# mryndzionek/composable-sdr

Measured on AMD Instinct MI355X. Metric: MS/s CF32 throughput, 256-ch PFB+FM pipeline, higher is better.
Workload: dtype f32; 1 GPU; cfg3: 256-ch firpfbch(m=7,As=80)+dcBlocker+freqdem(kf=0.3) on synthetic CF32, AGC off (-a 0), 262144 frames/step (512 MiB in, 256 MiB out), HBM-resident; channels=256, demod=fm, mix=False, route=fused-256|k_tile256<FM>, preheat_steps=12094, collective=none, rccl_ranks=1

## Files before the change

composable_sdr_amd/csrc/fused_common.h:

```cpp
#pragma once
#include "fused.h"
#include "run_split.h"

#include <cmath>
#include <cstdlib>
#include <vector>

namespace csdr {
namespace {

constexpr int M256 = 256;
constexpr int P = 14;
constexpr int NB = 16;
constexpr int FS_X = 272;
constexpr int FS_Z = 289;
constexpr int RS_Z = 18;
constexpr int RS_Y = 17;
constexpr int LDS_F2 = 16 * FS_Z;
constexpr int E_OFF = 4096;
constexpr int LOOKBACK = 10;
constexpr unsigned SPIN_LIMIT = 1u << 24;

typedef unsigned long long u64;
typedef float v2f __attribute__((ext_vector_type(2)));
// ... 327 lines not shown
    return f ? r : make_float2(0.f, 0.f);
}


constexpr int WU = 6;


struct RunArgs {
    TileArgs t;
    RunSplit split;
    PhaseK pk;
    uint32_t nruns;
    float l2beta;
    uint32_t prio_div;
    uint32_t trace_light;
    const float4 *prev_tail;
    uint32_t indep;
    uint32_t pair_align;
    uint32_t wu_batch6;
    uint32_t wu, wu_rot;
    uint32_t tile_step;
    uint32_t nowu;
    float2 *cpre, *side;
};
constexpr int DCFIX_F = 113;

__device__ __forceinline__ float2 wg_sum(float2 v, float2 *red, int tid)
{
#pragma unroll
    for (int d = 32; d >= 1; d >>= 1) { v.x += __shfl_xor(v.x, d); v.y += __shfl_xor(v.y, d); }
    if ((tid & 63) == 0) red[tid >> 6] = v;
    __syncthreads();
    const float2 r = cadd(cadd(red[0], red[1]), cadd(red[2], red[3]));
    __syncthreads();
    return r;
}

__device__ __forceinline__ void row_scan4(float &x0, float &x1, float &x2, float &x3, float &s0, float &s1, float &s2, float &s3,
                                          float b1, float b2, float b4, float b8, float na)
{
    asm volatile(
        "v_mov_b32_e32 %4, %0\n\t"
        "v_mov_b32_e32 %5, %1\n\t"
        "v_mov_b32_e32 %6, %2\n\t"
        "v_mov_b32_e32 %7, %3\n\t"
        "v_fmac_f32_dpp %4, %4, %8 row_shr:1 row_mask:0xf bank_mask:0xf\n\t"
        "v_fmac_f32_dpp %5, %5, %8 row_shr:1 row_mask:0xf bank_mask:0xf\n\t"
        "v_fmac_f32_dpp %6, %6, %8 row_shr:1 row_mask:0xf bank_mask:0xf\n\t"
// ... 72 lines not shown
```

composable_sdr_amd/csrc/fused_v2_common.h:

```cpp
#pragma once
#include "fused_common.h"

namespace csdr {
namespace {

typedef float v4f __attribute__((ext_vector_type(4)));
#ifndef V2_DMA_AUX
#define V2_DMA_AUX ""
#endif
#ifndef V2_DMA_AUX_STREAM
#define V2_DMA_AUX_STREAM V2_DMA_AUX
#endif

__device__ __forceinline__ void bar()
{
    asm volatile("s_waitcnt lgkmcnt(0)\n\ts_barrier" ::: "memory");
}
__device__ __forceinline__ float opaque_v(float x) { asm volatile("" : "+v"(x)); return x; }

__device__ __forceinline__ unsigned dma_offset(int tid)
{
    const int wave = tid >> 6, lane = tid & 63;
    const int slot = 64 * wave + lane, q = slot >> 3, i = (slot & 7) ^ ((q >> 1) & 7);
    return (unsigned)(8 * q + i) * 16u;
// ... 107 lines not shown
    const v2f wA = piv - uA, wB = piv - uB;
    m[0] = copysignf(sel_neg(q[0].x, wA.x, uA.x), q[0].y);
    m[1] = copysignf(sel_neg(q[1].x, wA.y, uA.y), q[1].y);
    m[2] = copysignf(sel_neg(q[2].x, wB.x, uB.x), q[2].y);
    m[3] = copysignf(sel_neg(q[3].x, wB.y, uB.y), q[3].y);
}

template <int CTRL> __device__ __forceinline__ float dpp_keep(float old, float v)
{
    return __int_as_float(__builtin_amdgcn_update_dpp(__float_as_int(old), __float_as_int(v), CTRL, 0xf, 0xf, false));
}

}
template <size_t OFF> __device__ __forceinline__ unsigned kernarg_u32_s()
{
    unsigned v = 0;
#if defined(__HIP_DEVICE_COMPILE__)
    typedef __attribute__((address_space(4))) const char *kptr;
    kptr ka = (kptr)__builtin_amdgcn_kernarg_segment_ptr();
    asm volatile("s_load_dword %0, %1, %2\n\ts_waitcnt lgkmcnt(0)" : "=s"(v) : "s"(ka), "n"(OFF) : "memory");
#endif
    return v;
}
template <size_t OFF> __device__ __forceinline__ float2 *kernarg_ptr_s()
{
    float2 *p = nullptr;
#if defined(__HIP_DEVICE_COMPILE__)
    typedef __attribute__((address_space(4))) const char *kptr;
    kptr ka = (kptr)__builtin_amdgcn_kernarg_segment_ptr();
    unsigned long long v;
    asm volatile("s_load_dwordx2 %0, %1, %2\n\ts_waitcnt lgkmcnt(0)" : "=s"(v) : "s"(ka), "n"(OFF) : "memory");
    p = reinterpret_cast<float2 *>(v);
#endif
    return p;
}

}
```

composable_sdr_amd/csrc/kernels_fused.hip:

```cpp
#include "fused_common.h"
#include <cstring>

namespace csdr {

namespace {

#define STAMP(i) do { if (A.trace && tid == 0) A.trace[(size_t)b * 16 + (i)] = __builtin_amdgcn_s_memtime(); } while (0)

template <bool FM>
__global__ __launch_bounds__(256) void k_tile256(TileArgs A)
{
    __shared__ __attribute__((aligned(16))) float2 R[LDS_F2];
    __shared__ float2 tw_s[M256];
    __shared__ float2 Tt[2][16];
    __shared__ float2 carry_s[2];
    __shared__ unsigned tile_s;

    const int tid = threadIdx.x;
    if (tid == 0) tile_s = atomicAdd(A.ticket, 1u);
    tw_s[tid] = A.tw[tid];
    __syncthreads();
    const unsigned b = tile_s;
    if (b >= A.nb) return;
    STAMP(0);
// ... 247 lines not shown

__global__ __launch_bounds__(64) void k_shard_gather(const float *__restrict__ src, float *__restrict__ dst, uint32_t c0, uint32_t G, uint32_t rem,
                                                     uint32_t nf, uint32_t t0, uint32_t w)
{
    const uint32_t m = blockIdx.x;
    for (uint32_t i = threadIdx.x; i < rem * w; i += 64) dst[((size_t)m * nf + t0) * w + i] = src[(size_t)(c0 + G * m) * rem * w + i];
}

constexpr float V2_WEIGHT_CF[8] = {1.2f, 0.8f, 1.f, 1.f, 1.f, 1.f, 1.f, 1.f};
constexpr float V2_WEIGHT_FM[8] = {1.24f, 0.76f, 1.f, 1.f, 1.f, 1.f, 1.f, 1.f};
constexpr float V2_WEIGHT_FM3[8] = {1.6f, 1.f, 0.6f, 1.f, 1.f, 1.f, 1.f, 1.f};
constexpr float EQUAL_WEIGHT[8] = {1.f, 1.f, 1.f, 1.f, 1.f, 1.f, 1.f, 1.f};

struct FusedPlan : ChainPlan {
    using ChainPlan::ChainPlan;
    std::string kernel;
    uint32_t max_nb = 0, epoch = 0;
    float *d_taps = nullptr;
    float2 *d_tw = nullptr, *d_wpre = nullptr;
    StreamState st;
    unsigned *d_ticket = nullptr, *d_yflag = nullptr, *d_status = nullptr;
    u64 *d_agg = nullptr, *d_ylast = nullptr;
    ColdStart cold;
    u64 *d_trace = nullptr;
    uint32_t run_min_tiles = 1024;
    float slot_weight[8] = {1.f, 1.f, 1.f, 1.f, 1.f, 1.f, 1.f, 1.f};
    uint32_t slot_pairs[8] = {0, 0, 0, 0, 0, 0, 0, 0};
    bool have_weights = false, have_pairs = false;
    bool pd_equal = false, pd_nocopy = false;
    uint32_t resident_wgs_v2 = 512;
    float *d_shard_tail = nullptr;
    float4 *d_tail[3] = {nullptr, nullptr, nullptr};
    int tail_w = 0;
    bool tail_valid = false, save_tails = false;
    TileArgs proto;
    RunArgs run_proto;

    int init();
    const char *name() const override { return kernel.c_str(); }
    bool tile_major_ok(uint32_t nf) const override;
    void keep_tail() override { save_tails = cfg.G == 1; }
    bool can_overlap(uint32_t nf) const override;
    bool tail_recorded() const override { return save_tails && tail_valid; }
    int status(unsigned *st) override;
    int trace(unsigned long long *out, uint32_t ntiles) override;
    int reset_state(hipStream_t s) override;
// ... 32 lines not shown
    if ((r = mem.alloc(&d_ticket, sizeof(unsigned)))) return r;
    if ((r = mem.alloc(&d_status, sizeof(unsigned)))) return r;
    if ((r = mem.alloc(&d_yflag, sizeof(unsigned) * max_nb))) return r;
    if ((r = mem.alloc(&d_agg, sizeof(u64) * 2 * max_nb))) return r;
    if ((r = mem.alloc(&d_ylast, sizeof(u64) * (size_t)cfg.M * max_nb))) return r;
    if (const char *e = diag_env("CSDR_RUN_MIN_TILES")) run_min_tiles = (uint32_t)atol(e);
    if (cfg.mix && (r = mem.alloc(&d_premix, (size_t)cfg.C * cfg.max_nf * (cfg.fm ? 4 : 8)))) return r;
    const char *trace_knob = diag_env("CSDR_TRACE");
    if (trace_knob) {
        if ((r = mem.alloc(&d_trace, sizeof(u64) * 16 * max_nb))) return r;
        CSDR_HIP(hipMemset(d_trace, 0, sizeof(u64) * 16 * max_nb));
    }
    CSDR_HIP(hipMemcpy(d_taps, cfg.taps, sizeof(float) * cfg.M * cfg.p, hipMemcpyHostToDevice));
    std::vector<float2> tw(cfg.M);
    for (uint32_t k1 = 0; k1 < 16; k1++)
        for (uint32_t b1 = 0; b1 < 16; b1++) {
            const double a = -2.0 * 3.14159265358979323846 * (double)(b1 * k1) / (double)cfg.M;
            tw[16 * k1 + b1] = make_float2((float)std::cos(a), (float)std::sin(a));
        }
    const std::vector<float2> wpre = premix_table();
    CSDR_HIP(hipMemcpy(d_tw, tw.data(), sizeof(float2) * cfg.M, hipMemcpyHostToDevice));
    CSDR_HIP(hipMemcpy(d_wpre, wpre.data(), sizeof(float2) * 2 * cfg.M, hipMemcpyHostToDevice));
    if (cfg.G == 1 && cfg.c0 == 0 && cfg.C == cfg.M &&
        (r = cold.init(mem, cfg, (DCFIX_F - 1) * 256.0, 2050, (size_t)2048 * 4 * DCFIX_F, false, 15u, (uint32_t)DCFIX_F, 126, wpre.data()))) return r;
    CSDR_HIP(hipMemset(d_status, 0, sizeof(unsigned)));
    CSDR_HIP(hipMemset(d_yflag, 0, sizeof(unsigned) * max_nb));
    CSDR_HIP(hipMemset(d_agg, 0, sizeof(u64) * 2 * max_nb));

    TileArgs &A = proto;
    A = TileArgs{};
    A.taps = d_taps; A.tw = d_tw; A.wpre = d_wpre;
    A.ticket = d_ticket; A.agg = d_agg; A.ylast = d_ylast; A.yflag = d_yflag; A.status = d_status;
    A.c0 = cfg.c0; A.C = cfg.C; A.fm_ref = cfg.fm_ref; A.trace = d_trace;
    dcc.put(A);
    if (const char *e = diag_env("CSDR_CUS")) { if (atoi(e) > 0 && (uint32_t)atoi(e) < cus) cus = (uint32_t)atoi(e); }
    resident_wgs_v2 = (uint32_t)(cus * run256_v2_blocks_per_cu(cfg.fm, cfg.G));
    if (const char *e = diag_env("CSDR_RESIDENT_WGS")) resident_wgs_v2 = (uint32_t)atol(e);
    if (const char *e = diag_env("CSDR_RUN_WEIGHTS")) { parse_list(e, slot_weight, atof); have_weights = true; }
    if (const char *e = diag_env("CSDR_RUN_PAIRS")) { parse_list(e, slot_pairs, atol); have_pairs = true; }
    pd_equal = diag_env("CSDR_PD_EQUAL") != nullptr;
    pd_nocopy = diag_env("CSDR_PD_NOCOPY") != nullptr;

    RunArgs &RA = run_proto;
    RA = RunArgs{};
    RA.pk = phase_consts(cfg.fm_ref);
    RA.l2beta = dcc.l2beta;
    RA.cpre = cold.cpre; RA.side = cold.side;
    { const char *e = diag_env("CSDR_PRIO_ROT"); RA.prio_div = (e && atoi(e)) ? cus : 0u; }
    RA.trace_light = (trace_knob && atoi(trace_knob) == 2) ? 1u : 0u;
    { const char *e = diag_env("CSDR_WU"); RA.wu = e ? (uint32_t)atoi(e) : (uint32_t)WU; }
    { const char *e = diag_env("CSDR_WU_ROT"); RA.wu_rot = e ? (uint32_t)atoi(e) : 0u; }
    RA.pair_align = (cfg.fm || diag_env("CSDR_PAIR_ALIGN_CF")) ? 1u : 0u;
    { const char *e = diag_env("CSDR_WU_BATCH6"); RA.wu_batch6 = e ? (uint32_t)atoi(e) : 1u; }
    return 0;
}

int FusedPlan::reset_state(hipStream_t s)
{
    if (int r = st.reset(s)) return r;
    CSDR_HIP(hipMemsetAsync(d_tail[0], 0, sizeof(float4) * 2048 * (WU + 1), s));
    tail_w = 0; tail_valid = true;
    return 0;
}

bool FusedPlan::tile_major_ok(uint32_t nf) const
{
    if (cfg.fm || cfg.mix || nf % NB || !nf) return false;
    if (cfg.G > 1) return (uint64_t)cfg.C * nf * 8u < (1ull << 32);
    return cfg.c0 == 0 && cfg.C == cfg.M && nf / NB >= run_min_tiles;
}

bool FusedPlan::can_overlap(uint32_t nf) const
{
    return save_tails && tail_valid && v2_call(nf) && nf % NB == 0 && !cfg.mix;
}

void FusedPlan::wire_state(TileArgs &A) const
{
    A.yhist_in = st.hist_in(cur); A.yhist_out = st.hist_out(cur);
    A.vend_in = st.vend_in(cur);  A.vend_out = st.vend_out(cur);
    A.rp_in = st.rp_in(cur);      A.rp_out = st.rp_out(cur);
}
// ... 25 lines not shown
    CSDR_HIP(hipGetLastError());
    return 0;
}

int FusedPlan::run_kernel(const FusedCall &call, const TileArgs &A, hipStream_t s, KernelTimer *timer)
{
    const FusedConfig &c = cfg;
    const bool shard = c.G > 1;
    int r;
    kernel = c.fm ? "k_run256v2<FM>" : "k_run256v2<CF32>";
    if (shard) kernel += "/G" + std::to_string(c.G);
    RunArgs RA = run_proto;
    RA.t = A;
    uint32_t nruns = resident_wgs_v2;
    if (nruns > A.nb / 8) nruns = A.nb / 8;
    if (nruns < 1) nruns = 1;
    RA.nruns = nruns;
    const float *v2_weight = c.fm ? ((cus && nruns == 3 * cus) ? V2_WEIGHT_FM3 : V2_WEIGHT_FM) : V2_WEIGHT_CF;
    RA.split = make_split(A.nb, nruns, cus, (call.indep && pd_equal) ? EQUAL_WEIGHT : (have_weights ? slot_weight : v2_weight),
                          have_pairs ? slot_pairs : nullptr);
    RA.tile_step = call.tile_major ? c.C * 128u : (uint32_t)NB * (c.fm ? 4u : 8u);
    RA.indep = call.indep ? 1u : 0u;
    RA.nowu = (cold.rt && !shard && !RA.indep && nruns >= 2 && nruns <= 2048) ? 1u : 0u;
    RA.prev_tail = d_tail[tail_w];
    if (save_tails && !shard && call.nf == A.nb * NB && A.nb >= WU + 1) {
        const int nxt = (tail_w + 1) % 3;
        if (!pd_nocopy) hipLaunchKernelGGL(k_save_tail, dim3(2048 * (WU + 1) / 256), dim3(256), 0, s,
                                           reinterpret_cast<const float4 *>(call.d_in + (size_t)(A.nb - (WU + 1)) * 4096), d_tail[nxt]);
        if (call.ev_tail) CSDR_HIP(hipEventRecord(call.ev_tail, s));
        tail_w = nxt; tail_valid = true;
    } else tail_valid = false;
    if (timer && (r = timer->begin(s))) return r;
    if (A.nb && (r = run256_v2_launch(&RA, c.fm, c.G, nruns, s))) return r;
    if (RA.nowu && A.nb && (r = run256_dcfix_launch(&RA, c.fm, nruns, cold.rt, s))) return r;
    if (timer && (r = timer->end(s))) return r;
    return 0;
}

int FusedPlan::tile_kernel(TileArgs &T, hipStream_t s, KernelTimer *timer)
{
    int r;
    if (++epoch == 0) epoch = 1;
    T.epoch = epoch;
    CSDR_HIP(hipMemsetAsync(d_ticket, 0, sizeof(unsigned), s));
    if (timer && (r = timer->begin(s))) return r;
    if (cfg.fm) hipLaunchKernelGGL(k_tile256<true>, dim3(T.nb), dim3(256), 0, s, T);
    else hipLaunchKernelGGL(k_tile256<false>, dim3(T.nb), dim3(256), 0, s, T);
    if (timer && (r = timer->end(s))) return r;
    return 0;
}

int FusedPlan::ragged_end(const FusedCall &call, void *out, uint32_t nb_full, uint32_t rem, hipStream_t s)
{
    const FusedConfig &c = cfg;
    const bool shard = c.G > 1;
    int r;
    if (nb_full) cur ^= 1;
    TileArgs T = proto;
// ... 30 lines not shown
```

composable_sdr_amd/csrc/kernels_fused_v2.hip:

```cpp
#ifndef V2_FM_PACKED
#define V2_FM_PACKED 1
#endif
#ifndef V2_ABLATE
#define V2_ABLATE 0
#endif

#ifndef V2_COLSCAN
#define V2_COLSCAN 0
#endif
#ifndef V2_PAIR
#define V2_PAIR 1
#endif
#ifndef V2_STORE_AUX
#define V2_STORE_AUX ""
#endif
#ifndef V2_PAIR_CF
#define V2_PAIR_CF 0
#endif
#ifndef V2_BAR_E
#define V2_BAR_E 0
#endif
#ifndef V2_PAD
#define V2_PAD 1
#endif
// ... 10 lines not shown
#include "fused_v2_common.h"
#include <cstddef>
#include <type_traits>

namespace csdr {
namespace {

constexpr unsigned V2_FSB = 2048u + (V2_PAD ? 128u : 0u);
constexpr int V2_FS2 = (int)V2_FSB / 8;
constexpr int V2_BUF = 16 * V2_FS2;
constexpr int V2_STASH = 2 * V2_BUF;
constexpr int V2_AUX2 = 256 + 32 + 256 + (V2_COLSCAN ? 512 : 0);
constexpr int V2_F2 = V2_STASH + V2_AUX2;
constexpr int V2_F2_ONE = V2_BUF + V2_AUX2 + P * M256 / 2;
#define V2_ZSW(f) (V2_PAD ? (((f) >> 1) & 7) : ((f) & 7))
#ifndef V2_RSWN
#define V2_RSWN V2_PAD
#endif
#define V2_RSW(a) (V2_RSWN ? ((a) & 7) : (((a) >> 1) & 7))

struct V2Args {
    RunArgs r;
};

template <bool FM, int G>
__global__ __launch_bounds__(256, (FM && G == 1) ? V2_ONE_WGS : 2) void k_run256v2(V2Args VA)
{
    static_assert(G == 1 || G == 2 || G == 4 || G == 8, "interleaved shards: G = 2, 4, 8");
    constexpr int NK1 = 16 / G;
    constexpr bool ONE = FM && G == 1;
    const RunArgs &RA = VA.r;
    const TileArgs &A = RA.t;
    __shared__ __attribute__((aligned(16))) float2 L[(ONE && V2_ONE_WGS >= 3) ? V2_F2_ONE : V2_F2];
    float2 *R = L, *ST = L + (ONE ? V2_BUF : V2_STASH), *Tt = ST + 256, *red = Tt + 16;
    float2 *tw_s = red + 16;
    float2 *TRc = tw_s + 256, *Ec = TRc + 256;
    (void)TRc; (void)Ec;
    float *TP = reinterpret_cast<float *>(L + (ONE ? V2_BUF : V2_STASH) + V2_AUX2);
    float2 *H = ONE ? L : L + V2_BUF;
    float2 *HS = ONE ? reinterpret_cast<float2 *>(TP) : H;
    float2 *E = ST;
    const int tid = threadIdx.x, j = tid;
    const unsigned w = blockIdx.x;
    unsigned first, last;
    run_range(RA.split, w, first, last);
    if (RA.pair_align) {
// ... 22 lines not shown
    const bool cold = w > 0 || RA.indep;
    const int halo = (int)first - 1;
    auto tile_ptr = [&](int t) -> const float4 * { return t >= 0 ? x4 + (size_t)t * 2048 : RA.prev_tail + (size_t)(WU + 1 + t) * 2048; };
    if (ONE) {
        if (cold) dma_tile<false, 2 * V2_FSB>(tile_ptr(halo), goff, lds_wave);
        else if (first < last) dma_tile<false, 2 * V2_FSB>(x4 + (size_t)first * 2048, goff, lds_wave);
    } else {
        if (first < last) dma_tile<false, 2 * V2_FSB>(x4 + (size_t)first * 2048, goff, lds_wave);
        if (cold) dma_tile<false, 2 * V2_FSB>(tile_ptr(halo), goff, lds_wave + (unsigned)(V2_BUF * 8));
    }
    float h[P];
#pragma unroll
    for (int n = 0; n < P; n++) h[n] = A.taps[(M256 - 1 - j) + n * M256];
    float2 Wa = A.wpre[(A.parity0 & 1) * M256 + j], Wb = A.wpre[((A.parity0 & 1) ^ 1) * M256 + j];
    if (G > 1) {
        const int n = ((j >> 4) * (int)A.c0) & 15;
        const float C1 = 0.92387953251128674f, S1 = 0.38268343236508977f, R2 = 0.70710678118654752f;
        const int m4 = n & 3, qd = n >> 2;
        const float2 e = m4 == 0 ? make_float2(1.f, 0.f) : (m4 == 1 ? make_float2(C1, -S1) : (m4 == 2 ? make_float2(R2, -R2) : make_float2(S1, -C1)));
        const float2 rot = qd == 0 ? e : (qd == 1 ? make_float2(e.y, -e.x) : (qd == 2 ? make_float2(-e.x, -e.y) : make_float2(-e.y, e.x)));
        Wa = cmul(Wa, rot); Wb = cmul(Wb, rot);
    }
    tw_s[tid] = A.tw[tid];
    float2 wa[NB], wb[NB];
#pragma unroll
    for (int f = 0; f < NB; f++) { wa[f] = make_float2(0.f, 0.f); wb[f] = make_float2(0.f, 0.f); }
    float2 c;
    float2 w2 = make_float2(0.f, 0.f);

    if (!cold) {
        c = A.vend_in[0];
#pragma unroll
        for (int f = 3; f < NB; f++) wa[f] = A.yhist_in[(f - 3) * M256 + j];
    } else {
        const int h0 = RA.nowu ? halo : (RA.indep ? halo - (int)RA.wu : (halo > (int)RA.wu ? halo - (int)RA.wu : 0));
        const unsigned nwu = (unsigned)(halo - h0);
        float4 raw[8];
        float wt0, wt1;
        {
            const int wave = tid >> 6, lane = tid & 63;
            const int slot = 64 * wave + lane, q = slot >> 3;
            const int i = (slot & 7) ^ ((q >> 1) & 7);
            const int n = 16 * q + 2 * i;
            wt0 = exp2f((float)(4095 - n) * RA.l2beta);
            wt1 = exp2f((float)(4094 - n) * RA.l2beta);
        }
// ... 73 lines not shown
            const float2 s2 = (n == P - 1) ? w2 : wa[NB - 1 - n];
            acc = __builtin_elementwise_fma((v2f){s2.x, s2.y}, (v2f){h[n], h[n]}, acc);
        }
        HS[j] = to_f2(acc);
        __syncthreads();
        v2f vv[16];
        if (tid < 16) {
#pragma unroll
            for (int a = 0; a < 16; a++) vv[a] = to_v(HS[16 * a + tid]);
            fft16_v(vv);
#pragma unroll
            for (int i = (G > 1 ? 0 : 1); i < 16; i++) vv[i] = cmul_v(vv[i], to_v(tw_s[16 * ((XIDX(i) + (G > 1 ? (int)A.c0 : 0)) & 15) + tid]));
#pragma unroll
            for (int i = 0; i < 16; i++) HS[256 + 16 * XIDX(i) + tid] = to_f2(vv[i]);
        }
        __syncthreads();
        if (tid < 16) {
#pragma unroll
            for (int b = 0; b < 16; b++) vv[b] = to_v(HS[256 + 16 * (G * (tid % NK1)) + b]);
            fft16_v(vv);
#pragma unroll
            for (int i = 0; i < 16; i++) ST[tid * 16 + i] = to_f2(vv[i]);
            if (G == 1 && RA.nowu) {
                if (tid >= 14) RA.side[((size_t)w * 4 + (tid - 14)) * DCFIX_F] = to_f2(vv[13]);
                else if (tid <= 1) RA.side[((size_t)w * 4 + 2 + tid) * DCFIX_F] = to_f2(vv[2]);
            }
        }
        __syncthreads();
    }

    if (ONE) {
#pragma unroll
        for (int n = 0; n < P; n++) TP[M256 * n + j] = h[n];
    }
    const v2f Wav = to_v(Wa), Wbv = to_v(Wb);
    const float na = opaque_v(-A.alpha), be = opaque_v(A.beta);
    const float kJ = -A.alpha * exp2f((float)j * RA.l2beta);
    const float b256 = A.b256[1];
    const FmK2 fk = {{opaque_v(9.999993443e-01f), opaque_v(-3.332985938e-01f), opaque_v(1.994656026e-01f), opaque_v(-1.390860826e-01f),
                      opaque_v(9.642146528e-02f), opaque_v(-5.591168255e-02f), opaque_v(2.186254039e-02f), opaque_v(-4.054457881e-03f)},
                     opaque_v(1e-37f), opaque_v(A.fm_ref), opaque_v(RA.pk.hp), opaque_v(RA.pk.pi)};
    const int q = tid, sw = V2_RSW(q & 15);
    const unsigned raw_a_ = (unsigned)q * 128u + (unsigned)(q >> 4) * (V2_FSB - 2048u) + ((unsigned)sw << 4);
    const int f1 = tid >> 4, b1 = tid & 15;
    const int k1 = tid >> 4, f2 = tid & 15;
    const unsigned x_a_ = (unsigned)f1 * V2_FSB + (unsigned)b1 * 8u;
    const unsigned zw_a = (unsigned)f1 * V2_FSB + (unsigned)((((b1 >> 1) ^ V2_ZSW(f1)) << 1) | (b1 & 1)) * 8u;
    const unsigned z_a_ = (unsigned)f2 * V2_FSB + (unsigned)k1 * 128u + ((unsigned)V2_ZSW(f2) << 4);
// ... 1 lines not shown
    const unsigned z_a_g = (unsigned)f2 * V2_FSB + (unsigned)(G * j1) * 128u + ((unsigned)V2_ZSW(f2) << 4);
    const uint32_t voff = ((uint32_t)(G == 1 ? k1 : j1 + 16 * hb) * A.out_stride + A.out_t0 + (uint32_t)f2) * (FM ? 4u : 8u);
    const size_t row16 = (size_t)NK1 * A.out_stride * (FM ? 4u : 8u);
#if V2_TRACE
#define V2STAMP(i) do { if (A.trace && !RA.trace_light && tid == 0) A.trace[(size_t)b_ * 16 + (i)] = __builtin_amdgcn_s_memtime(); } while (0)
#else
#define V2STAMP(i) do { } while (0)
#endif

    float hold[16];
    v2f holdc[V2_PAIR_CF ? 16 : 1];
    auto tile = [&](float2 (&old)[NB], float2 (&nw)[NB], unsigned b_, const int par) {
        unsigned b = (unsigned)__builtin_amdgcn_readfirstlane((int)b_);
        asm volatile("" : "+s"(b));
        char *B = reinterpret_cast<char *>(L) + (ONE ? 0 : par) * (V2_BUF * 8);
        float2 *Bf = reinterpret_cast<float2 *>(B);
        if (RA.prio_div) {
            if (((b_ - first) + w / RA.prio_div) & 1u) __builtin_amdgcn_s_setprio(1); else __builtin_amdgcn_s_setprio(0);
        }
        int tid_t = tid;
        if (ONE) asm volatile("" : "+v"(tid_t));
        V2STAMP(0);
        if (G == 1 && b + 1 == last && tid == 0) {
            if (kernarg_u32_s<offsetof(V2Args, r.nowu)>()) kernarg_ptr_s<offsetof(V2Args, r.cpre)>()[w + 1] = c;
        }
        if (V2_TRACE && A.trace && !RA.trace_light && tid == 0) A.trace[(size_t)b_ * 16 + 15] = __builtin_amdgcn_s_memrealtime();
        bar();
        V2STAMP(1);
#ifdef V2_SELECTIVE_POLICY
        if (!(V2_ABLATE & 1) && b + 1 < last) {
            if (b + 1 + (WU + 1) < last) dma_tile<true, 2 * V2_FSB>(x4 + (size_t)(b + 1) * 2048, goff, lds_wave + (unsigned)(par ^ 1) * (V2_BUF * 8u));
            else dma_tile<false, 2 * V2_FSB>(x4 + (size_t)(b + 1) * 2048, goff, lds_wave + (unsigned)(par ^ 1) * (V2_BUF * 8u));
        }
#else
        if (!ONE && !(V2_ABLATE & 1) && b + 1 < last) dma_tile<false, 2 * V2_FSB>(x4 + (size_t)(b + 1) * 2048, goff, lds_wave + (unsigned)(par ^ 1) * (V2_BUF * 8u));
#endif
        auto next_pieces = [&](const int it) {
            if (ONE && !(V2_ABLATE & 1) && b + 1 < last) {
                dma_piece<2 * V2_FSB>(x4 + (size_t)(b + 1) * 2048, goff, lds_wave, it);
                dma_piece<2 * V2_FSB>(x4 + (size_t)(b + 1) * 2048, goff, lds_wave, it + 1);
            }
        };
#if V2_COLSCAN
#pragma unroll
        for (int f = 0; f < NB; f++) nw[f] = Bf[V2_FS2 * f + col_off];
        col_run_scan(nw, TRc, A, tid);
        V2STAMP(2);
        bar();
        col_run_carries(TRc, Ec, Tt, A, tid);
        bar();
        V2STAMP(3);
// ... 182 lines not shown
            if (G == 2) { if (wave_u < 2u) shard_tail(std::integral_constant<int, 0>{}); else shard_tail(std::integral_constant<int, 2>{}); }
            else switch (wave_u) {
                case 0: shard_tail(std::integral_constant<int, 0>{}); break;
                case 1: shard_tail(std::integral_constant<int, 1>{}); break;
                case 2: shard_tail(std::integral_constant<int, 2>{}); break;
                default: shard_tail(std::integral_constant<int, 3>{}); break;
            }
            V2STAMP(14);
            return;
        }
        const unsigned z_a = ONE ? (unsigned)(tid_t & 15) * V2_FSB + (unsigned)(tid_t >> 4) * 128u + ((unsigned)V2_ZSW(tid_t & 15) << 4) : z_a_;
#pragma unroll
        for (int i = 0; i < 8; i++) {
            const v4f v = *reinterpret_cast<const v4f *>(B + (z_a ^ (unsigned)(i << 4)));
            vv[2 * i] = (v2f){v.x, v.y}; vv[2 * i + 1] = (v2f){v.z, v.w};
        }
        if (ONE) {
            bar();
            next_pieces(0);
            if (V2_ONE_BURST) { next_pieces(2); next_pieces(4); next_pieces(6); }
        }
        if (!(V2_ABLATE & 16)) fft16_v(vv);
        V2STAMP(11);
        if (G == 1 && cold && b - first < 7u && kernarg_u32_s<offsetof(V2Args, r.nowu)>()) {
            const int k1s = ONE ? tid_t >> 4 : k1, f2s = ONE ? tid_t & 15 : f2;
            float2 *sd = kernarg_ptr_s<offsetof(V2Args, r.side)>() + ((size_t)w * 4) * DCFIX_F + 1 + 16 * (size_t)(b - first) + f2s;
            if (k1s >= 14) sd[(k1s - 14) * DCFIX_F] = to_f2(vv[13]);
            else if (k1s <= 1) sd[(2 + k1s) * DCFIX_F] = to_f2(vv[2]);
        }
        char *obase = reinterpret_cast<char *>(A.out) + (size_t)b * RA.tile_step;
        if (FM) {
            if (!ONE) asm volatile("s_waitcnt vmcnt(0)" ::: "memory");
#pragma unroll
            for (int i = 0; i < 16; i += 4) {
                float2 rp[4], rr[4];
#pragma unroll
                for (int u = 0; u < 4; u += 2) {
                    const v4f sp = *reinterpret_cast<const v4f *>(ST + k1 * 16 + i + u);
                    rp[u] = make_float2(dpp_keep<0x111>(sp.x, vv[i + u].x), dpp_keep<0x111>(sp.y, vv[i + u].y));
                    rp[u + 1] = make_float2(dpp_keep<0x111>(sp.z, vv[i + u + 1].x), dpp_keep<0x111>(sp.w, vv[i + u + 1].y));
                    rr[u] = to_f2(vv[i + u]); rr[u + 1] = to_f2(vv[i + u + 1]);
                }
                float mq_[4];
                float (&mq)[4] = (V2_PAIR && par == 0) ? *reinterpret_cast<float (*)[4]>(&hold[i]) : mq_;
                if (V2_ABLATE & 4) { mq[0] = rp[0].x + rr[0].y; mq[1] = rp[1].y + rr[1].x; mq[2] = rp[2].x + rr[2].y; mq[3] = rp[3].y + rr[3].x; }
                else if (V2_FM_PACKED) fm_quad(rp, rr, fk, mq);
                else {
                    const FmK k1s = {fk.tiny, fk.ref, fk.hp, fk.pi};
#pragma unroll
                    for (int u = 0; u < 4; u++) mq[u] = fm_sample(rp[u], rr[u], k1s);
                }
                if (!V2_ONE_BURST && i < 12) next_pieces(2 + i / 2);
                if (V2_PAIR && par == 0 && b + 1 < last) continue;
#pragma unroll
                for (int u = 0; u < 4; u++) {
                    const char *rowp = obase + (size_t)XIDX(i + u) * row16;
                    if (V2_ABLATE & 2) asm volatile("" :: "v"(mq[u]), "s"(rowp));
                    else {
                        if (V2_PAIR && par == 1) asm volatile(V2_SNOP "global_store_dword %0, %1, %2 offset:-64" V2_STORE_AUX :: "v"(voff), "v"(hold[i + u]), "s"(rowp) : "memory");
                        asm volatile(V2_SNOP "global_store_dword %0, %1, %2" V2_STORE_AUX :: "v"(voff), "v"(mq[u]), "s"(rowp) : "memory");
                    }
                }
            }
            if (f2 == 15) {
#pragma unroll
                for (int i = 0; i < 16; i += 2) *reinterpret_cast<v4f *>(ST + k1 * 16 + i) = (v4f){vv[i].x, vv[i].y, vv[i + 1].x, vv[i + 1].y};
            }
            if (ONE && b + 1 < last) {
                if ((V2_PAIR && par == 0) || (V2_ABLATE & 2)) asm volatile("s_waitcnt vmcnt(0)" ::: "memory");
                else asm volatile("s_waitcnt vmcnt(%0)" :: "n"((V2_ONE_BURST ? 4 : 2) * (V2_PAIR ? 8 : 4)) : "memory");
            }
            V2STAMP(12);
            V2STAMP(13);
        } else {
            V2STAMP(12);
            asm volatile("s_waitcnt vmcnt(0)" ::: "memory");
            V2STAMP(13);
            if (V2_PAIR_CF && par == 0 && b + 1 < last) {
#pragma unroll
                for (int i = 0; i < 16; i++) holdc[i] = vv[i];
            } else {
#pragma unroll
                for (int i = 0; i < 16; i++) {
                    const char *rowp = obase + (size_t)XIDX(i) * row16;
                    if (V2_ABLATE & 2) asm volatile("" :: "v"(vv[i]), "s"(rowp));
                    else {
                        if (V2_PAIR_CF && par == 1) asm volatile(V2_SNOP "global_store_dwordx2 %0, %1, %2 offset:-128" V2_STORE_AUX :: "v"(voff), "v"(holdc[i]), "s"(rowp) : "memory");
                        asm volatile(V2_SNOP "global_store_dwordx2 %0, %1, %2" V2_STORE_AUX :: "v"(voff), "v"(vv[i]), "s"(rowp) : "memory");
                    }
                }
            }
        }
        V2STAMP(14);
    };

    V2LSTAMP(2);
    asm volatile("s_waitcnt vmcnt(0)" ::: "memory");
    V2LSTAMP(3);
    for (unsigned b = first; b < last; b += 2) {
        tile(wa, wb, b, 0);
        if (b + 1 >= last) break;
        tile(wb, wa, b + 1, 1);
    }

    V2LSTAMP(4);
    bar();
    if (FM) {
        const float2 lastY = ST[st_idx];
        if (last == A.nb && st_own) A.rp_out[tid] = lastY;
    }
    if (last == A.nb && tid == 0) A.vend_out[0] = c;
}

}

template <bool FM>
__global__ __launch_bounds__(128) void k_run256_dcfix(V2Args VA, const float2 *__restrict__ Rt)
{
    const RunArgs &RA = VA.r;
    const TileArgs &A = RA.t;
    __shared__ float2 Ys[4][DCFIX_F + 1];
    const unsigned w = blockIdx.x + 1;
    unsigned first, last;
    run_range(RA.split, w, first, last);
    if (RA.pair_align) { first &= ~1u; if (last != A.nb) last &= ~1u; }
    if (first >= last || first <= 1) return;
    const int t = threadIdx.x;
    const float2 c = RA.cpre[w];
    const float2 *R = Rt + (size_t)(A.parity0 & 1u) * DCFIX_F * 4;
    float2 y[4];
    if (t < DCFIX_F) {
#pragma unroll
        for (int ch = 0; ch < 4; ch++) {
            const float2 r = R[t * 4 + ch], s0 = RA.side[((size_t)w * 4 + ch) * DCFIX_F + t];
            y[ch] = make_float2(fmaf(c.x, r.x, fmaf(-c.y, r.y, s0.x)), fmaf(c.x, r.y, fmaf(c.y, r.x, s0.y)));
            Ys[ch][t] = y[ch];
        }
    }
    __syncthreads();
    if (t < 1 || t >= DCFIX_F) return;
    const unsigned b = first + (unsigned)(t - 1) / 16u, f2 = (unsigned)(t - 1) & 15u;
    if (b >= last) return;
    char *obase = reinterpret_cast<char *>(A.out) + (size_t)b * RA.tile_step;
    const FmK fk = {1e-37f, A.fm_ref, RA.pk.hp, RA.pk.pi};
#pragma unroll
    for (int ch = 0; ch < 4; ch++) {
        const size_t off = ((size_t)(126 + ch) * A.out_stride + A.out_t0 + f2) * (FM ? 4u : 8u);
        if (FM) *reinterpret_cast<float *>(obase + off) = fm_sample(Ys[ch][t - 1], y[ch], fk);
        else *reinterpret_cast<float2 *>(obase + off) = y[ch];
    }
}

int run256_dcfix_launch(const void *run_args, bool fm, unsigned nruns, const float2 *Rt, hipStream_t s)
{
    if (nruns < 2) return 0;
    V2Args VA;
    VA.r = *static_cast<const RunArgs *>(run_args);
    if (fm) hipLaunchKernelGGL(k_run256_dcfix<true>, dim3(nruns - 1), dim3(128), 0, s, VA, Rt);
    else hipLaunchKernelGGL(k_run256_dcfix<false>, dim3(nruns - 1), dim3(128), 0, s, VA, Rt);
    return 0;
}

static V2Args make_v2(const void *run_args)
{
    V2Args VA;
    VA.r = *static_cast<const RunArgs *>(run_args);
    return VA;
}

int run256_v2_launch(const void *run_args, bool fm, unsigned G, unsigned nruns, hipStream_t s)
{
    const V2Args VA = make_v2(run_args);
#define V2_LAUNCH(F, GG) hipLaunchKernelGGL((k_run256v2<F, GG>), dim3(nruns), dim3(256), 0, s, VA)
    if (G == 1) { if (fm) V2_LAUNCH(true, 1); else V2_LAUNCH(false, 1); }
    else if (G == 2) { if (fm) V2_LAUNCH(true, 2); else V2_LAUNCH(false, 2); }
    else if (G == 4) { if (fm) V2_LAUNCH(true, 4); else V2_LAUNCH(false, 4); }
    else if (G == 8) { if (fm) V2_LAUNCH(true, 8); else V2_LAUNCH(false, 8); }
    else { set_error("k_run256v2: interleaved shards of stride %u are not built (2, 4, 8)", G); return -1; }
#undef V2_LAUNCH
    return 0;
}

// ... 12 lines not shown
```

Measured before the change: 320,400 MS/s.

## Fuse DC-fix pass into main FM kernel via per-run ticket handoff

Removes the separate k_run256_dcfix launch in the FM path by having each workgroup of the main kernel do the boundary correction itself. A per-run atomic ticket counter pairs the producer of the carry (previous run's end state) with the consumer (next run's first tiles), and whichever workgroup arrives second applies the fix. Side and cpre data are written with system-coherent stores so they are visible across workgroups. The fix window is widened from 7 to 8 tiles, and the affected output slots are skipped in the main store path. This trades a kernel launch and tail pass for extra atomics, an added vmcnt drain at the end of every workgroup, and more complex cross-workgroup ordering.

```diff
diff --git a/composable_sdr_amd/csrc/fused_common.h b/composable_sdr_amd/csrc/fused_common.h
--- a/composable_sdr_amd/csrc/fused_common.h
+++ b/composable_sdr_amd/csrc/fused_common.h
@@ -373,8 +373,14 @@
     uint32_t tile_step;
     uint32_t nowu;
     float2 *cpre, *side;
+    uint32_t fuse;
+    unsigned *tk;
+    const float2 *rt;
 };
-constexpr int DCFIX_F = 113;
+constexpr int DCFIX_F = 129;
+constexpr int DCFIX_TILES = (DCFIX_F - 1) / 16;
+constexpr int DCFIX_SIDE = (4 * DCFIX_F + 15) / 16 * 16;
+constexpr int CPRE_STRIDE = 16;
 
 __device__ __forceinline__ float2 wg_sum(float2 v, float2 *red, int tid)
 {
diff --git a/composable_sdr_amd/csrc/fused_v2_common.h b/composable_sdr_amd/csrc/fused_v2_common.h
--- a/composable_sdr_amd/csrc/fused_v2_common.h
+++ b/composable_sdr_amd/csrc/fused_v2_common.h
@@ -153,15 +153,15 @@
 #endif
     return v;
 }
-template <size_t OFF> __device__ __forceinline__ float2 *kernarg_ptr_s()
+template <size_t OFF, class T = float2> __device__ __forceinline__ T *kernarg_ptr_s()
 {
-    float2 *p = nullptr;
+    T *p = nullptr;
 #if defined(__HIP_DEVICE_COMPILE__)
     typedef __attribute__((address_space(4))) const char *kptr;
     kptr ka = (kptr)__builtin_amdgcn_kernarg_segment_ptr();
     unsigned long long v;
     asm volatile("s_load_dwordx2 %0, %1, %2\n\ts_waitcnt lgkmcnt(0)" : "=s"(v) : "s"(ka), "n"(OFF) : "memory");
-    p = reinterpret_cast<float2 *>(v);
+    p = reinterpret_cast<T *>(v);
 #endif
     return p;
 }
diff --git a/composable_sdr_amd/csrc/kernels_fused.hip b/composable_sdr_amd/csrc/kernels_fused.hip
--- a/composable_sdr_amd/csrc/kernels_fused.hip
+++ b/composable_sdr_amd/csrc/kernels_fused.hip
@@ -293,6 +293,8 @@
     unsigned *d_ticket = nullptr, *d_yflag = nullptr, *d_status = nullptr;
     u64 *d_agg = nullptr, *d_ylast = nullptr;
     ColdStart cold;
+    unsigned *d_tk = nullptr;
+    bool dcfix_launch = false;
     u64 *d_trace = nullptr;
     uint32_t run_min_tiles = 1024;
     float slot_weight[8] = {1.f, 1.f, 1.f, 1.f, 1.f, 1.f, 1.f, 1.f};
@@ -371,7 +373,10 @@
     CSDR_HIP(hipMemcpy(d_tw, tw.data(), sizeof(float2) * cfg.M, hipMemcpyHostToDevice));
     CSDR_HIP(hipMemcpy(d_wpre, wpre.data(), sizeof(float2) * 2 * cfg.M, hipMemcpyHostToDevice));
     if (cfg.G == 1 && cfg.c0 == 0 && cfg.C == cfg.M &&
-        (r = cold.init(mem, cfg, (DCFIX_F - 1) * 256.0, 2050, (size_t)2048 * 4 * DCFIX_F, false, 15u, (uint32_t)DCFIX_F, 126, wpre.data()))) return r;
+        (r = cold.init(mem, cfg, (DCFIX_F - 1) * 256.0, (size_t)2050 * CPRE_STRIDE, (size_t)2048 * DCFIX_SIDE, false, 15u, (uint32_t)DCFIX_F, 126, wpre.data()))) return r;
+    if ((r = mem.alloc(&d_tk, sizeof(unsigned) * 2049))) return r;
+    CSDR_HIP(hipMemset(d_tk, 0, sizeof(unsigned) * 2049));
+    { const char *e = diag_env("CSDR_DCFIX_LAUNCH"); dcfix_launch = e && atoi(e) != 0; }
     CSDR_HIP(hipMemset(d_status, 0, sizeof(unsigned)));
     CSDR_HIP(hipMemset(d_yflag, 0, sizeof(unsigned) * max_nb));
     CSDR_HIP(hipMemset(d_agg, 0, sizeof(u64) * 2 * max_nb));
@@ -394,7 +399,7 @@
     RA = RunArgs{};
     RA.pk = phase_consts(cfg.fm_ref);
     RA.l2beta = dcc.l2beta;
-    RA.cpre = cold.cpre; RA.side = cold.side;
+    RA.cpre = cold.cpre; RA.side = cold.side; RA.rt = cold.rt; RA.tk = d_tk;
     { const char *e = diag_env("CSDR_PRIO_ROT"); RA.prio_div = (e && atoi(e)) ? cus : 0u; }
     RA.trace_light = (trace_knob && atoi(trace_knob) == 2) ? 1u : 0u;
     { const char *e = diag_env("CSDR_WU"); RA.wu = e ? (uint32_t)atoi(e) : (uint32_t)WU; }
@@ -407,6 +412,7 @@
 int FusedPlan::reset_state(hipStream_t s)
 {
     if (int r = st.reset(s)) return r;
+    CSDR_HIP(hipMemsetAsync(d_tk, 0, sizeof(unsigned) * 2049, s));
     CSDR_HIP(hipMemsetAsync(d_tail[0], 0, sizeof(float4) * 2048 * (WU + 1), s));
     tail_w = 0; tail_valid = true;
     return 0;
@@ -478,6 +484,8 @@
     RA.tile_step = call.tile_major ? c.C * 128u : (uint32_t)NB * (c.fm ? 4u : 8u);
     RA.indep = call.indep ? 1u : 0u;
     RA.nowu = (cold.rt && !shard && !RA.indep && nruns >= 2 && nruns <= 2048) ? 1u : 0u;
+    RA.fuse = (RA.nowu && c.fm && !dcfix_launch) ? 1u : 0u;
+    if (RA.nowu && c.fm && dcfix_launch) kernel += "+k_run256_dcfix<FM>";
     RA.prev_tail = d_tail[tail_w];
     if (save_tails && !shard && call.nf == A.nb * NB && A.nb >= WU + 1) {
         const int nxt = (tail_w + 1) % 3;
@@ -488,8 +496,17 @@
     } else tail_valid = false;
     if (timer && (r = timer->begin(s))) return r;
     if (A.nb && (r = run256_v2_launch(&RA, c.fm, c.G, nruns, s))) return r;
-    if (RA.nowu && A.nb && (r = run256_dcfix_launch(&RA, c.fm, nruns, cold.rt, s))) return r;
+    if (RA.nowu && !RA.fuse && A.nb && (r = run256_dcfix_launch(&RA, c.fm, nruns, cold.rt, s))) return r;
     if (timer && (r = timer->end(s))) return r;
+#ifdef CSDR_DEBUG_TICKETS
+    if (RA.fuse && A.nb) {
+        std::vector<unsigned> tk(nruns + 1);
+        CSDR_HIP(hipStreamSynchronize(s));
+        CSDR_HIP(hipMemcpy(tk.data(), d_tk, sizeof(unsigned) * tk.size(), hipMemcpyDeviceToHost));
+        for (uint32_t v = 0; v <= nruns; v++)
+            if (tk[v] & 1u) { set_error("k_run256v2: ticket %u of %u is odd (%u) behind the launch", v, nruns, tk[v]); return -1; }
+    }
+#endif
     return 0;
 }
 
diff --git a/composable_sdr_amd/csrc/kernels_fused_v2.hip b/composable_sdr_amd/csrc/kernels_fused_v2.hip
--- a/composable_sdr_amd/csrc/kernels_fused_v2.hip
+++ b/composable_sdr_amd/csrc/kernels_fused_v2.hip
@@ -56,6 +56,60 @@
 struct V2Args {
     RunArgs r;
 };
+
+__device__ __forceinline__ void side_store(float2 *p, v2f v)
+{
+    asm volatile("global_store_dwordx2 %0, %1, off sc0 sc1" :: "v"(p), "v"(v) : "memory");
+}
+__device__ __forceinline__ void side_store(float2 *p, float2 v) { side_store(p, to_v(v)); }
+
+template <bool FM, bool SC1, int NT, class RAP>
+__device__ __forceinline__ void dcfix_apply(RAP ra, const float2 *__restrict__ Rt, unsigned w, unsigned first, unsigned last,
+                                            float2 *Ys, int tid)
+{
+    constexpr int NE = 4 * DCFIX_F, NI = (NE + NT - 1) / NT;
+    static_assert(NI <= 3, "dcfix_apply: at most three elements per thread");
+    const float2 *cp = ra->cpre + (size_t)w * CPRE_STRIDE;
+    const float2 *sd = ra->side + (size_t)w * DCFIX_SIDE;
+    const float2 *R = Rt + (size_t)(ra->t.parity0 & 1u) * DCFIX_F * 4;
+    v2f sv[3], cv;
+    const float2 *sp[3];
+#pragma unroll
+    for (int i = 0; i < 3; i++) { const int e = tid + NT * i; sp[i] = sd + (e < NE ? e : NE - 1); }
+    if (SC1) {
+        asm volatile("global_load_dwordx2 %0, %4, off sc1\n\tglobal_load_dwordx2 %1, %5, off sc1\n\tglobal_load_dwordx2 %2, %6, off sc1\n\t"
+                     "global_load_dwordx2 %3, %7, off sc1\n\ts_waitcnt vmcnt(0)"
+                     : "=&v"(sv[0]), "=&v"(sv[1]), "=&v"(sv[2]), "=&v"(cv) : "v"(sp[0]), "v"(sp[1]), "v"(sp[2]), "v"(cp) : "memory");
+    } else {
+#pragma unroll
+        for (int i = 0; i < 3; i++) sv[i] = to_v(*sp[i]);
+        cv = to_v(*cp);
+    }
+    const float2 c = to_f2(cv);
+#pragma unroll
+    for (int i = 0; i < NI; i++) {
+        const int e = tid + NT * i;
+        if (e < NE) {
+            const int ch = e / DCFIX_F, t = e - ch * DCFIX_F;
+            const float2 r = R[t * 4 + ch], s0 = to_f2(sv[i]);
+            Ys[e] = make_float2(fmaf(c.x, r.x, fmaf(-c.y, r.y, s0.x)), fmaf(c.x, r.y, fmaf(c.y, r.x, s0.y)));
+        }
+    }
+    __syncthreads();
+    const FmK fk = {1e-37f, ra->t.fm_ref, ra->pk.hp, ra->pk.pi};
+    char *const out = reinterpret_cast<char *>(ra->t.out);
+    const uint32_t tile_step = ra->tile_step, out_stride = ra->t.out_stride, out_t0 = ra->t.out_t0;
+    for (int e = tid; e < 4 * (DCFIX_F - 1); e += NT) {
+        const int ch = e / (DCFIX_F - 1), t = 1 + e % (DCFIX_F - 1);
+        const unsigned b = first + (unsigned)(t - 1) / 16u, f2 = (unsigned)(t - 1) & 15u;
+        if (b >= last) continue;
+        char *o = out + (size_t)b * tile_step + ((size_t)(126 + ch) * out_stride + out_t0 + f2) * (FM ? 4u : 8u);
+        const float2 y = Ys[ch * DCFIX_F + t];
+        if (FM) *reinterpret_cast<float *>(o) = fm_sample(Ys[ch * DCFIX_F + t - 1], y, fk);
+        else *reinterpret_cast<float2 *>(o) = y;
+    }
+    __syncthreads();
+}
 
 template <bool FM, int G>
 __global__ __launch_bounds__(256, (FM && G == 1) ? V2_ONE_WGS : 2) void k_run256v2(V2Args VA)
@@ -124,6 +178,9 @@
         Wa = cmul(Wa, rot); Wb = cmul(Wb, rot);
     }
     tw_s[tid] = A.tw[tid];
+    typedef __attribute__((address_space(1))) unsigned *tk_ptr;
+    unsigned *fix_me = reinterpret_cast<unsigned *>(red + 8);
+    if (ONE && tid == 0) *fix_me = 0u;
     float2 wa[NB], wb[NB];
 #pragma unroll
     for (int f = 0; f < NB; f++) { wa[f] = make_float2(0.f, 0.f); wb[f] = make_float2(0.f, 0.f); }
@@ -243,8 +300,8 @@
 #pragma unroll
             for (int i = 0; i < 16; i++) ST[tid * 16 + i] = to_f2(vv[i]);
             if (G == 1 && RA.nowu) {
-                if (tid >= 14) RA.side[((size_t)w * 4 + (tid - 14)) * DCFIX_F] = to_f2(vv[13]);
-                else if (tid <= 1) RA.side[((size_t)w * 4 + 2 + tid) * DCFIX_F] = to_f2(vv[2]);
+                if (tid >= 14) side_store(RA.side + (size_t)w * DCFIX_SIDE + (tid - 14) * DCFIX_F, vv[13]);
+                else if (tid <= 1) side_store(RA.side + (size_t)w * DCFIX_SIDE + (2 + tid) * DCFIX_F, vv[2]);
             }
         }
         __syncthreads();
@@ -292,11 +349,18 @@
         if (ONE) asm volatile("" : "+v"(tid_t));
         V2STAMP(0);
         if (G == 1 && b + 1 == last && tid == 0) {
-            if (kernarg_u32_s<offsetof(V2Args, r.nowu)>()) kernarg_ptr_s<offsetof(V2Args, r.cpre)>()[w + 1] = c;
+            if (kernarg_u32_s<offsetof(V2Args, r.nowu)>()) side_store(kernarg_ptr_s<offsetof(V2Args, r.cpre)>() + (size_t)(w + 1) * CPRE_STRIDE, c);
         }
         if (V2_TRACE && A.trace && !RA.trace_light && tid == 0) A.trace[(size_t)b_ * 16 + 15] = __builtin_amdgcn_s_memrealtime();
         bar();
         V2STAMP(1);
+        if (ONE && cold && b - first == (unsigned)DCFIX_TILES && first > 1u && kernarg_u32_s<offsetof(V2Args, r.fuse)>()) {
+            if (tid == 0) {
+                asm volatile("s_waitcnt vmcnt(0)" ::: "memory");
+                const unsigned old = __hip_atomic_fetch_add((tk_ptr)kernarg_ptr_s<offsetof(V2Args, r.tk), unsigned>() + w, 1u, __ATOMIC_RELAXED, __HIP_MEMORY_SCOPE_AGENT);
+                if (old & 1u) *fix_me = 1u;
+            }
+        }
 #ifdef V2_SELECTIVE_POLICY
         if (!(V2_ABLATE & 1) && b + 1 < last) {
             if (b + 1 + (WU + 1) < last) dma_tile<true, 2 * V2_FSB>(x4 + (size_t)(b + 1) * 2048, goff, lds_wave + (unsigned)(par ^ 1) * (V2_BUF * 8u));
@@ -525,11 +589,11 @@
         }
         if (!(V2_ABLATE & 16)) fft16_v(vv);
         V2STAMP(11);
-        if (G == 1 && cold && b - first < 7u && kernarg_u32_s<offsetof(V2Args, r.nowu)>()) {
+        if (G == 1 && cold && b - first < (unsigned)DCFIX_TILES && kernarg_u32_s<offsetof(V2Args, r.nowu)>()) {
             const int k1s = ONE ? tid_t >> 4 : k1, f2s = ONE ? tid_t & 15 : f2;
-            float2 *sd = kernarg_ptr_s<offsetof(V2Args, r.side)>() + ((size_t)w * 4) * DCFIX_F + 1 + 16 * (size_t)(b - first) + f2s;
-            if (k1s >= 14) sd[(k1s - 14) * DCFIX_F] = to_f2(vv[13]);
-            else if (k1s <= 1) sd[(2 + k1s) * DCFIX_F] = to_f2(vv[2]);
+            float2 *sd = kernarg_ptr_s<offsetof(V2Args, r.side)>() + (size_t)w * DCFIX_SIDE + 1 + 16 * (size_t)(b - first) + f2s;
+            if (k1s >= 14) side_store(sd + (k1s - 14) * DCFIX_F, vv[13]);
+            else if (k1s <= 1) side_store(sd + (2 + k1s) * DCFIX_F, vv[2]);
         }
         char *obase = reinterpret_cast<char *>(A.out) + (size_t)b * RA.tile_step;
         if (FM) {
@@ -558,11 +622,16 @@
 #pragma unroll
                 for (int u = 0; u < 4; u++) {
                     const char *rowp = obase + (size_t)XIDX(i + u) * row16;
-                    if (V2_ABLATE & 2) asm volatile("" :: "v"(mq[u]), "s"(rowp));
-                    else {
+                    auto store_slot = [&]() {
                         if (V2_PAIR && par == 1) asm volatile(V2_SNOP "global_store_dword %0, %1, %2 offset:-64" V2_STORE_AUX :: "v"(voff), "v"(hold[i + u]), "s"(rowp) : "memory");
                         asm volatile(V2_SNOP "global_store_dword %0, %1, %2" V2_STORE_AUX :: "v"(voff), "v"(mq[u]), "s"(rowp) : "memory");
-                    }
+                    };
+                    if (V2_ABLATE & 2) asm volatile("" :: "v"(mq[u]), "s"(rowp));
+                    else if (ONE && (i + u == 13 || i + u == 2) && cold && b - first < (unsigned)DCFIX_TILES && first > 1u &&
+                             kernarg_u32_s<offsetof(V2Args, r.fuse)>()) {
+                        const int k1s = tid_t >> 4;
+                        if (i + u == 13 ? k1s < 14 : k1s > 1) store_slot();
+                    } else store_slot();
                 }
             }
             if (f2 == 15) {
@@ -607,51 +676,61 @@
     }
 
     V2LSTAMP(4);
+    if (ONE) asm volatile("s_waitcnt vmcnt(0)" ::: "memory");
     bar();
     if (FM) {
         const float2 lastY = ST[st_idx];
         if (last == A.nb && st_own) A.rp_out[tid] = lastY;
     }
     if (last == A.nb && tid == 0) A.vend_out[0] = c;
+    if (ONE && kernarg_u32_s<offsetof(V2Args, r.fuse)>()) {
+        typedef __attribute__((address_space(4))) const RunArgs *rap_t;
+        rap_t rp = (rap_t)((__attribute__((address_space(4))) const char *)__builtin_amdgcn_kernarg_segment_ptr() + offsetof(V2Args, r));
+        asm volatile("" : "+s"(rp));
+        const float2 *rt = rp->rt;
+        const unsigned nb = rp->t.nb;
+        unsigned f_ = first, l_ = last;
+        asm volatile("" : "+s"(f_), "+s"(l_));
+        unsigned fn = 0, ln = 0;
+        const unsigned nruns = kernarg_u32_s<offsetof(V2Args, r.nruns)>();
+        const bool nxt = w + 1 < nruns;
+        if (nxt) {
+            const unsigned rps = rp->split.rps, s = (w + 1) / rps, i = (w + 1) - s * rps, base = rp->split.base[s], tiles = rp->split.tiles[s];
+            const unsigned sh = rp->split.shift, n = tiles >> sh;
+            fn = base + ((unsigned)((unsigned long long)i * n / rps) << sh);
+            ln = base + (i + 1 == rps ? tiles : ((unsigned)((unsigned long long)(i + 1) * n / rps) << sh));
+            if (rp->pair_align) { fn &= ~1u; if (ln != nb) ln &= ~1u; }
+        }
+        if (tid == 0) {
+            unsigned m = *fix_me;
+            tk_ptr tk = (tk_ptr)kernarg_ptr_s<offsetof(V2Args, r.tk), unsigned>();
+            if (cold && f_ > 1u && f_ < l_ && l_ - f_ <= (unsigned)DCFIX_TILES)
+                m = __hip_atomic_fetch_add(tk + w, 1u, __ATOMIC_RELAXED, __HIP_MEMORY_SCOPE_AGENT) & 1u;
+            if (nxt && fn > 1u && fn < ln)
+                m |= (__hip_atomic_fetch_add(tk + w + 1, 1u, __ATOMIC_RELAXED, __HIP_MEMORY_SCOPE_AGENT) & 1u) << 1;
+            *fix_me = m;
+        }
+        __syncthreads();
+        const unsigned m = *fix_me;
+        if (m & 1u) dcfix_apply<true, true, 256>(rp, rt, w, f_, l_, L, tid);
+        if (m & 2u) dcfix_apply<true, true, 256>(rp, rt, w + 1, fn, ln, L, tid);
+    }
 }
 
 }
 
 template <bool FM>
-__global__ __launch_bounds__(128) void k_run256_dcfix(V2Args VA, const float2 *__restrict__ Rt)
+__global__ __launch_bounds__(256) void k_run256_dcfix(V2Args VA, const float2 *__restrict__ Rt)
 {
     const RunArgs &RA = VA.r;
     const TileArgs &A = RA.t;
-    __shared__ float2 Ys[4][DCFIX_F + 1];
+    __shared__ float2 Ys[4 * DCFIX_F];
     const unsigned w = blockIdx.x + 1;
     unsigned first, last;
     run_range(RA.split, w, first, last);
     if (RA.pair_align) { first &= ~1u; if (last != A.nb) last &= ~1u; }
     if (first >= last || first <= 1) return;
-    const int t = threadIdx.x;
-    const float2 c = RA.cpre[w];
-    const float2 *R = Rt + (size_t)(A.parity0 & 1u) * DCFIX_F * 4;
-    float2 y[4];
-    if (t < DCFIX_F) {
-#pragma unroll
-        for (int ch = 0; ch < 4; ch++) {
-            const float2 r = R[t * 4 + ch], s0 = RA.side[((size_t)w * 4 + ch) * DCFIX_F + t];
-            y[ch] = make_float2(fmaf(c.x, r.x, fmaf(-c.y, r.y, s0.x)), fmaf(c.x, r.y, fmaf(c.y, r.x, s0.y)));
-            Ys[ch][t] = y[ch];
-        }
-    }
-    __syncthreads();
-    if (t < 1 || t >= DCFIX_F) return;
-    const unsigned b = first + (unsigned)(t - 1) / 16u, f2 = (unsigned)(t - 1) & 15u;
-    if (b >= last) return;
-    char *obase = reinterpret_cast<char *>(A.out) + (size_t)b * RA.tile_step;
-    const FmK fk = {1e-37f, A.fm_ref, RA.pk.hp, RA.pk.pi};
-#pragma unroll
-    for (int ch = 0; ch < 4; ch++) {
-        const size_t off = ((size_t)(126 + ch) * A.out_stride + A.out_t0 + f2) * (FM ? 4u : 8u);
-        if (FM) *reinterpret_cast<float *>(obase + off) = fm_sample(Ys[ch][t - 1], y[ch], fk);
-        else *reinterpret_cast<float2 *>(obase + off) = y[ch];
-    }
+    dcfix_apply<FM, false, 256>(&RA, Rt, w, first, last, Ys, (int)threadIdx.x);
 }
 
 int run256_dcfix_launch(const void *run_args, bool fm, unsigned nruns, const float2 *Rt, hipStream_t s)
@@ -659,8 +738,8 @@
     if (nruns < 2) return 0;
     V2Args VA;
     VA.r = *static_cast<const RunArgs *>(run_args);
-    if (fm) hipLaunchKernelGGL(k_run256_dcfix<true>, dim3(nruns - 1), dim3(128), 0, s, VA, Rt);
-    else hipLaunchKernelGGL(k_run256_dcfix<false>, dim3(nruns - 1), dim3(128), 0, s, VA, Rt);
+    if (fm) hipLaunchKernelGGL(k_run256_dcfix<true>, dim3(nruns - 1), dim3(256), 0, s, VA, Rt);
+    else hipLaunchKernelGGL(k_run256_dcfix<false>, dim3(nruns - 1), dim3(256), 0, s, VA, Rt);
     return 0;
 }
 
```

New measurement: 321,800 MS/s (median of 5 runs). No clear change (+0.4%).
